# HaiminLuo/svox_t

Hardware: AMD Instinct MI355X
Metric: Mrays/s fwd+bwd, 800×800 render, depth-8 SH9 N3Tree, 1→8 MI355X (higher is better)
Workload: dtype f32

## Files before the change

### svox_t_amd/csrc/svoxt_bwd.hip

```cpp

#include <hip/hip_runtime.h>
#include <stdint.h>

#include "svoxt_launch.h"

#pragma clang fp contract(off)

#include "svoxt_bwd_kernels.h"

using namespace svoxt;

namespace {
int64_t* g_bwd_counters = nullptr;
int64_t* g_bwd_check = nullptr;

template <bool REPLAY>
bool launch_bwd_xform(const TreeDev& tr, const RaysDev& rays, const Opts& opt, int C,
                      const float* grad_out, float* grad, int gstride, RecLists L, const uint4* aux,
                      const float* fwd_out, hipStream_t st) {
    if (opt.format != FMT_SH || C != 3) return false;
    const unsigned nb = nblocks(rays.Q);
#define SVOXT_BWD_XF(BB)                                                                                      \
    hipLaunchKernelGGL((render_bwd_kernel<FMT_SH, 3, BB, true, REPLAY, true>), dim3(nb), dim3(kBlock), 0, st, \
                       tr, rays, opt, grad_out, grad, gstride, L, aux, fwd_out);                         \
    return true;
    switch (opt.basis_dim) {
        case 1: SVOXT_BWD_XF(1)
        case 4: SVOXT_BWD_XF(4)
        case 9: SVOXT_BWD_XF(9)
        case 16: SVOXT_BWD_XF(16)
        case 25: SVOXT_BWD_XF(25)
    }
#undef SVOXT_BWD_XF
    return false;
}

bool launch_lobes_bwd_tiles(const TreeDev& tr, const RaysDev& rays, const Opts& opt, const float* grad_out, float* grad,
                            int gstride, RecLists L, const uint4* aux, hipStream_t st, int terms_state) {
    if (L.terms == nullptr || terms_state != 3 || !lobes_payload(opt, tr.K) || g_bwd_counters != nullptr) return false;
    const unsigned nb = nblocks(rays.Q);
#define SVOXT_LOBES_BWD(BB)                                                                                         \
    {                                                                                                               \
        hipLaunchKernelGGL((render_bwd_kernel<FMT_SH, 3, BB, true, true, false, true, false, true>), dim3(nb), dim3(kBlock), \
                           0, st, tr, rays, opt, grad_out, grad, gstride, L, aux, (const float*)nullptr, (float4*)nullptr); \
        hipLaunchKernelGGL((grad_fused_kernel<FMT_SH, BB, true, false, 3, true>), dim3(nb), dim3(512), 0, st,       \
                           tr, rays, opt, grad_out, L, aux, (const float*)nullptr, grad, gstride);                  \
        return true;                                                                                                \
    }
    switch (opt.basis_dim) {
        case 1: SVOXT_LOBES_BWD(1)
        case 4: SVOXT_LOBES_BWD(4)
        case 9: SVOXT_LOBES_BWD(9)
        case 16: SVOXT_LOBES_BWD(16)
        case 25: SVOXT_LOBES_BWD(25)
    }
#undef SVOXT_LOBES_BWD
    return false;
}

bool launch_bwd_gather(const TreeDev& tr, const RaysDev& rays, const Opts& opt, int C,
                       const float* grad_out, float* grad, int gstride, RecLists L, const uint4* aux,
                       const float* fwd_out, float4* coef, bool xf, hipStream_t st, int terms_state = 0,
                       bool native = false) {
    const unsigned nb = nblocks(rays.Q);
    if (C > 3) {
        if (opt.format != FMT_RGBA || coef != nullptr || xf || fwd_out != nullptr || L.terms == nullptr) return false;
#define SVOXT_WIDE(KK)                                                                                        \
    {                                                                                                         \
        hipLaunchKernelGGL((render_bwd_kernel<FMT_RGBA, KK - 1, 0, true, true, false, true>), dim3(nb), dim3(kBlock), 0, st, \
                           tr, rays, opt, grad_out, grad, gstride, L, aux, (const float*)nullptr, (float4*)nullptr); \
        unsigned long long* ctr = reinterpret_cast<unsigned long long*>(g_bwd_counters);                      \
        unsigned long long* chkw = reinterpret_cast<unsigned long long*>(g_bwd_check);                        \
        if (chkw != nullptr && !native)                                                                       \
            hipLaunchKernelGGL((grad_wide_kernel<KK, false, false, true>), dim3(nb), dim3(512), 0, st, tr, rays, opt, grad_out, L, aux, \
                               grad, gstride, chkw);                                                          \
        else if (chkw != nullptr)                                                                             \
            return false;                                                                                     \
        else if (ctr != nullptr)                                                                              \
// ... 7 lines not shown
                               grad, gstride, (unsigned long long*)nullptr);                                  \
        else                                                                                                  \
            hipLaunchKernelGGL((grad_wide_kernel<KK, false>), dim3(nb), dim3(512), 0, st, tr, rays, opt, grad_out, L, aux, \
                               grad, gstride, (unsigned long long*)nullptr);                                  \
        return true;                                                                                          \
    }
        if (C == 7 && tr.K == 8) SVOXT_WIDE(8)
        if (C == 15 && tr.K == 16) SVOXT_WIDE(16)
        if (C == 31 && tr.K == 32) SVOXT_WIDE(32)
#undef SVOXT_WIDE
        return false;
    }
    if (C != 3) return false;
    const bool fused = coef == nullptr;
    if (fused && xf && (fwd_out != nullptr || opt.format != FMT_SH || opt.basis_dim > 9)) return false;
#define SVOXT_GATHER(F, BB)                                                                                   \
    if (fused) {    \
        hipLaunchKernelGGL((render_bwd_kernel<F, 3, BB, true, true, false, true>), dim3(nb), dim3(kBlock), 0, st, \
                           tr, rays, opt, grad_out, grad, gstride, L, aux, fwd_out, (float4*)nullptr);   \
        unsigned long long* ctr = reinterpret_cast<unsigned long long*>(g_bwd_counters);                      \
        unsigned long long* chkw = reinterpret_cast<unsigned long long*>(g_bwd_check);                        \
        if (chkw != nullptr) {     \
            if (L.terms != nullptr && terms_state == 3 && fwd_out == nullptr)                                 \
                hipLaunchKernelGGL((grad_fused_kernel<F, BB, true, false, 3, false, true>), dim3(nb), dim3(512), 0, st, \
                                   tr, rays, opt, grad_out, L, aux, fwd_out, grad, gstride, chkw);            \
            else if constexpr (F == FMT_SH && BB == 9) {                                                      \
                if (fwd_out != nullptr)                                                                       \
                    hipLaunchKernelGGL((grad_fused_kernel<F, BB, false, false, 0, false, true>), dim3(nb), dim3(512), 0, st, \
                                       tr, rays, opt, grad_out, L, aux, fwd_out, grad, gstride, chkw);        \
                else if (L.terms != nullptr && terms_state == 2)                                              \
                    hipLaunchKernelGGL((grad_fused_kernel<F, BB, true, false, 2, false, true>), dim3(nb), dim3(512), 0, st, \
                                       tr, rays, opt, grad_out, L, aux, fwd_out, grad, gstride, chkw);        \
                else                                                                                          \
                    hipLaunchKernelGGL((grad_fused_kernel<F, BB, true, false, 0, false, true>), dim3(nb), dim3(512), 0, st, \
                                       tr, rays, opt, grad_out, L, aux, fwd_out, grad, gstride, chkw); \
            } else return false;                                                                              \
            return true;                                                                                      \
        }                                                                                                     \
        if (fwd_out != nullptr && ctr == nullptr)                                                             \
            hipLaunchKernelGGL((grad_fused_kernel<F, BB, false>), dim3(nb), dim3(512), 0, st,                 \
                               tr, rays, opt, grad_out, L, aux, fwd_out, grad, gstride);                 \
        else if (ctr == nullptr && L.terms != nullptr && terms_state == 2)                                    \
            hipLaunchKernelGGL((grad_fused_kernel<F, BB, true, false, 2>), dim3(nb), dim3(512), 0, st,        \
                               tr, rays, opt, grad_out, L, aux, fwd_out, grad, gstride);                      \
        else if (ctr == nullptr && L.terms != nullptr && terms_state == 3)                                    \
            hipLaunchKernelGGL((grad_fused_kernel<F, BB, true, false, 3>), dim3(nb), dim3(512), 0, st,        \
                               tr, rays, opt, grad_out, L, aux, fwd_out, grad, gstride);                      \
        else if (ctr == nullptr)            \
            hipLaunchKernelGGL((grad_fused_kernel<F, BB, true>), dim3(nb), dim3(512), 0, st,                  \
                               tr, rays, opt, grad_out, L, aux, fwd_out, grad, gstride);                 \
        else if (fwd_out != nullptr)                                                                          \
            hipLaunchKernelGGL((grad_fused_kernel<F, BB, false, true>), dim3(nb), dim3(512), 0, st,           \
                               tr, rays, opt, grad_out, L, aux, fwd_out, grad, gstride, ctr);            \
        else                                                                                                  \
            hipLaunchKernelGGL((grad_fused_kernel<F, BB, true, true>), dim3(nb), dim3(512), 0, st,            \
                               tr, rays, opt, grad_out, L, aux, fwd_out, grad, gstride, ctr);            \
        return true;                                                                                          \
    }                                                                                                         \
    hipLaunchKernelGGL((render_bwd_kernel<F, 3, BB, true, true, false, true>), dim3(nb), dim3(kBlock), 0, st, \
                       tr, rays, opt, grad_out, grad, gstride, L, aux, fwd_out, coef);                   \
    hipLaunchKernelGGL((grad_merge_kernel<F, BB, 1024, 1024, 4>), dim3(nb), dim3(256), 0, st, tr, rays,      \
                       grad_out, L, coef, aux, grad, gstride);                                                \
    return true;
#define SVOXT_GATHER_XF(BB)                                                                                       \
    hipLaunchKernelGGL((render_bwd_kernel<FMT_SH, 3, BB, true, true, true, true>), dim3(nb), dim3(kBlock), 0, st, \
                       tr, rays, opt, grad_out, grad, gstride, L, aux, fwd_out, coef);                       \
    hipLaunchKernelGGL((grad_merge_kernel<FMT_SH, BB, 1024, 512, 4, true>), dim3(nb), dim3(256), 0, st, tr, rays, \
                       grad_out, L, coef, aux, grad, gstride);                                                    \
    return true;
#define SVOXT_FUSED_XF(BB)                                                                                        \
    {                                                                                                             \
// ... 18 lines not shown
            return false;
        }
        switch (opt.basis_dim) {
            case 1: SVOXT_GATHER_XF(1)
            case 4: SVOXT_GATHER_XF(4)
            case 9: SVOXT_GATHER_XF(9)
        }
        return false;
    }
#undef SVOXT_FUSED_XF
    if (opt.format == FMT_RGBA) { SVOXT_GATHER(FMT_RGBA, 0) }
#define SVOXT_GATHER_WIDE(BB)                                                                                 \
    {                                                                                                         \
        if (!fused || g_bwd_counters != nullptr || fwd_out != nullptr || L.terms == nullptr ||                \
            (terms_state != 2 && terms_state != 3)) return false;                                             \
        hipLaunchKernelGGL((render_bwd_kernel<FMT_SH, 3, BB, true, true, false, true>), dim3(nb), dim3(kBlock), 0, st, \
                           tr, rays, opt, grad_out, grad, gstride, L, aux, fwd_out, (float4*)nullptr);        \
        unsigned long long* chkw = reinterpret_cast<unsigned long long*>(g_bwd_check);                        \
        if (chkw != nullptr && terms_state == 2)                                                              \
            return false;                                                                                     \
        else if (chkw != nullptr)                                                                             \
            hipLaunchKernelGGL((grad_fused_kernel<FMT_SH, BB, true, false, 3, false, true>), dim3(nb), dim3(512), 0, st, \
                               tr, rays, opt, grad_out, L, aux, fwd_out, grad, gstride, chkw);                \
        else if (terms_state == 2)                                                                            \
            hipLaunchKernelGGL((grad_fused_kernel<FMT_SH, BB, true, false, 2>), dim3(nb), dim3(512), 0, st,   \
                               tr, rays, opt, grad_out, L, aux, fwd_out, grad, gstride);                      \
        else                                                                                                  \
            hipLaunchKernelGGL((grad_fused_kernel<FMT_SH, BB, true, false, 3>), dim3(nb), dim3(512), 0, st,   \
                               tr, rays, opt, grad_out, L, aux, fwd_out, grad, gstride);                      \
        return true;                                                                                          \
    }
    if (opt.format == FMT_SH) {
        switch (opt.basis_dim) {
            case 1: SVOXT_GATHER(FMT_SH, 1)
            case 4: SVOXT_GATHER(FMT_SH, 4)
            case 9: SVOXT_GATHER(FMT_SH, 9)
            case 16: SVOXT_GATHER_WIDE(16)
            case 25: SVOXT_GATHER_WIDE(25)
        }
    }
#undef SVOXT_GATHER_WIDE
#undef SVOXT_GATHER
#undef SVOXT_GATHER_XF
    return false;
// ... 107 lines not shown
        }
        else
            done = launch_bwd_xform<false>(tr, rd, od, C, grad_out, grad_features, gs,
                                           dense_lists(S > 0 ? workspace : nullptr, S, rays->Q), nullptr, nullptr, st);
    } else if (C > 0 && full_comp(opt) && !xf)
    {
        const int64_t S = workspace != nullptr ? rec_capacity(workspace_bytes, rays->Q) : 0;
        const RecLists wl = dense_lists(S > 0 ? workspace : nullptr, S, rays->Q);
        if (lists != nullptr) {
            const bool wide = opt->format == SVOXT_FORMAT_RGBA && C > 3;
            const RecLists ll = lists_dev(lists, rays->Q, wide ? 8 : 16);
            const RecLists l1 = wide ? lists_dev(lists, rays->Q, 4) : ll;
            const uint4* laux = reinterpret_cast<const uint4*>(lists->aux);
            if (lobes_payload(od, tree->K)) {
                if (n2 && lists->coef_bytes < 0)
                    done = launch_lobes_bwd_tiles(tr, rd, od, grad_out, grad_features, gs, ll, laux, st, lists->terms_state);
                if (!done) return fail(SVOXT_ERR_UNSUPPORTED, "%s: SG / ASG sample lists serve the per-tile backward only (N = 2, lists.terms filled by the forward: terms_state 3, coef_bytes < 0)", fn);
                return check_launch(fn);
            }
            const bool have_coef = lists->coef != nullptr &&
                                   lists->coef_bytes >= (int64_t)lists->max_samples * rays->Q * 16;
            if (n2 && (tree->K <= 32 || !have_coef) && (have_coef || lists->coef_bytes < 0))
                done = launch_bwd_gather(tr, rd, od, C, grad_out, grad_features, gs, ll, laux,
                                         fwd_out, have_coef ? reinterpret_cast<float4*>(lists->coef) : nullptr, false, st,
                                         (lists->terms_state == 2 || lists->terms_state == 3) ? lists->terms_state : 1,
                                         (lists->flags & SVOXT_LISTS_NATIVE_MATH) != 0);
            if (!done) done = n2 ? launch_bwd_special<true, true>(tr, rd, od, C, grad_out, grad_features, gs, l1, laux, fwd_out, st)
                      : launch_bwd_special<false, true>(tr, rd, od, C, grad_out, grad_features, gs, l1, laux, fwd_out, st);
            if (!done) return fail(SVOXT_ERR_UNSUPPORTED, "%s: no specialised kernel for this payload", fn);
        } else {
            done = n2 ? launch_bwd_special<true, false>(tr, rd, od, C, grad_out, grad_features, gs, wl, nullptr, nullptr, st)
                      : launch_bwd_special<false, false>(tr, rd, od, C, grad_out, grad_features, gs, wl, nullptr, nullptr, st);
        }
    } else if (lists != nullptr) {
        return fail(SVOXT_ERR_UNSUPPORTED, "%s: sample lists need a specialised payload", fn);
    }
    if (!done) {
        const unsigned nb = nblocks(rays->Q);
        const size_t lds = (size_t)(kBlock / 64) * 64 * (tree->K | 1) * sizeof(float) + kBlock * sizeof(int32_t);
        if (C > 0 && lds <= 65536) {
            if (n2) hipLaunchKernelGGL((render_bwd_generic_staged_kernel<true>), dim3(nb), dim3(kBlock), lds, st, tr, rd, od, C, grad_out, grad_features, gs);
// ... 25 lines not shown
```

### svox_t_amd/csrc/svoxt_bwd_kernels.h

```cpp
#pragma once

#include <hip/hip_runtime.h>
#include <stdint.h>

#include "svoxt_device.h"
#include "svoxt_lists.h"

#pragma clang fp contract(off)

#ifndef SVOXT_WIDE_STAGE_ROWS
#define SVOXT_WIDE_STAGE_ROWS 2
#endif
#ifndef SVOXT_WIDE_XCD_ROWS
#define SVOXT_WIDE_XCD_ROWS 1
#endif
#ifndef SVOXT_WIDE_ETAB_WAVES
#define SVOXT_WIDE_ETAB_WAVES 8
#endif

namespace svoxt {



template <int FMT, int C, int BD, int K, bool XF = false>
// ... 180 lines not shown
                  float4* __restrict__ coef_out = nullptr) {
    static_assert(!GATHER || (REPLAY && (C == 3 || FMT == FMT_RGBA)), "per-tile backward: lists; 3 channels or RGBA-style rows");
    static_assert(!ONEPASS || (REPLAY && FMT == FMT_RGBA && !XF && !GATHER), "one sigmoid pass: RGBA-style rows, lists");
    constexpr int K = (FMT == FMT_RGBA) ? (C + 1) : (C * BD + 1);
    constexpr int KS = K | 1;
    __shared__ float stage_all[(kBlock / 64) * 64 * KS];
    __shared__ int32_t sidx_all[kBlock];
    __shared__ uint2 rstage[REPLAY ? 1 : kRecBlock * kBlock];
    __shared__ int32_t ltab[REPLAY ? 1 : kMaxRecBlocks];
    if constexpr (!REPLAY) rec_tab_init(ltab);
    uint2* __restrict__ rec = L.rec;
    const int S = L.S;
    int64_t cur_block = 0;

    if constexpr (GATHER) {
        if (coef_out == nullptr && no_ray_overflowed(L)) return;
    }
    const bool only_overflowed = XF && REPLAY && !GATHER && reinterpret_cast<uintptr_t>(coef_out) == kOnlyOverflowed;
    if (only_overflowed && no_ray_overflowed(L)) return;
    const int lane = threadIdx.x & 63;
    float* stage = stage_all + (threadIdx.x >> 6) * (64 * KS);
    int32_t* sidx = sidx_all + (threadIdx.x >> 6) * 64;
    const unsigned long long lane_lt = (1ull << lane) - 1ull;
    const int64_t tid = (int64_t)blockIdx.x * kBlock + threadIdx.x;
    const int64_t q = ray_of_thread(rays, tid);
    Ray r;
    bool alive = q < rays.Q;
    if (only_overflowed) alive = alive && (aux[alive ? q : 0].x & kRecOverflow) != 0u;
    if constexpr (GATHER) {
        if (coef_out == nullptr && !__any(alive && (aux[alive ? q : 0].x & kRecOverflow) != 0u)) return;
// ... 438 lines not shown
            __builtin_amdgcn_wave_barrier();
        }
        if (k0 + RPP * kRound >= maxn) break;
        __syncthreads();
        for (int i = threadIdx.x; i < T; i += NT) { keys[i] = -1; cnt[i] = 0; }
        if (threadIdx.x == 0) s_nb = 0;
        __syncthreads();
    }
}

template <int FMT, int BD, bool EXACT, bool COUNT = false, int TERMS = 0, bool LOBES = false, bool CHECK = false, bool XF = false>
__global__ void __launch_bounds__(512, 4)
grad_fused_kernel(TreeDev tr, RaysDev rays, Opts opt, const float* __restrict__ grad_out,
                  RecLists L, const uint4* __restrict__ aux, const float* __restrict__ fwd_out,
                  float* __restrict__ grad, int gstride, unsigned long long* __restrict__ counters = nullptr) {
    if (tile_never_recorded(L, blockIdx.x)) return;
#define SVOXT_CHK(i, n, site) chk<CHECK>(i, n, counters, site)
    float4* __restrict__ terms = L.terms;
    constexpr int C = 3, W = 8, P = W - 1, NT = 64 * W, T = 1024, R = (FMT == FMT_SH && BD > 16) ? 896 : 1024;
    static_assert(2 * P * 64 <= R && P >= 1 && P <= W && R <= T, "a pair of rounds must fit the record arrays, a pass the hash table");
    constexpr int K = (FMT == FMT_RGBA) ? (C + 1) : (C * BD + 1);
    constexpr int NB = (FMT == FMT_SH) ? BD : 0;
    constexpr int BDS = (FMT == FMT_SH) ? (BD | 1) : 1;
    constexpr int HALF = K < 16 ? K : 16;
    constexpr int NH = (K + HALF - 1) / HALF;
    constexpr int KS = HALF | 1;
    static_assert(TERMS == 0 || TERMS == 2 || TERMS == 3, "hand-over layouts");
    static_assert(K <= 32 || (EXACT && TERMS >= 2), "wide rows: only with the forward's hand-over (no row in registers)");
    static_assert(!LOBES || (FMT == FMT_SH && EXACT && TERMS >= 2), "lobes: only over the forward's hand-over");
    static_assert(!XF || (FMT == FMT_SH && EXACT && (TERMS == 0 || TERMS == 3) && !LOBES && BD <= 9), "view rotations: SH rows in registers, exact");
    __shared__ float vds[XF ? 64 * 3 : 1];
    __shared__ int32_t keys[T];
    __shared__ int32_t cnt[T];
    __shared__ uint16_t order[R];
    __shared__ uint32_t r_sl[R];
    __shared__ float r_sg[R], r_w[R], r_c[3 * R], r_dt[R];
    __shared__ float bases[64 * BDS];
    __shared__ float gl[64 * 3];
    __shared__ float stage_all[W * 64 * KS];
    __shared__ int32_t seg_all[W * 64];
    __shared__ int32_t s_nb;
    const int lane = threadIdx.x & 63, wave = __builtin_amdgcn_readfirstlane((int)(threadIdx.x >> 6));
    const int pw = wave - (W - P);
    float* stage = stage_all + wave * 64 * KS;
    int32_t* seg = seg_all + wave * 64;
    const int32_t tabreg = rec_tab_reg(L, blockIdx.x, lane);
    const int64_t q = ray_of_thread(rays, (int64_t)blockIdx.x * 64 + lane);
    const bool in_batch = q < rays.Q;
    const int64_t qc = in_batch ? q : 0;
    const bool from_tensors = rays.c2w == nullptr;
    uint4 a = aux[qc];
    float g[C + 1], dsrc[3] = {0.f, 0.f, 1.f}, vsrc[3] = {0.f, 0.f, 1.f};
    if (from_tensors) {
#pragma unroll
        for (int j = 0; j < 3; ++j) dsrc[j] = rays.dirs[3 * qc + j];
        if constexpr (FMT == FMT_SH) {
#pragma unroll
            for (int j = 0; j < 3; ++j) vsrc[j] = rays.vdirs[3 * qc + j];
        }
    }
#pragma unroll
    for (int j = 0; j <= C; ++j) g[j] = grad_out[qc * (C + 1) + j];
    for (int i = threadIdx.x; i < T; i += NT) { keys[i] = -1; cnt[i] = 0; }
    if (!in_batch) a = make_uint4(0u, 0u, 0u, 0u);
    if constexpr (XF) { if (a.x & kRecOverflow) a.x = 0u; }
    const int nrec = (int)(a.x & ~kRecOverflow);
    int maxn = nrec;
    for (int off = 32; off > 0; off >>= 1) maxn = max(maxn, __shfl_xor(maxn, off, 64));
    maxn = __builtin_amdgcn_readfirstlane(maxn);
    if (maxn == 0) return;
    if constexpr (CHECK) { if (threadIdx.x == 0) atomicAdd(counters + kChkBase + 29, 1ull); }

    Ray r;
    float basis[NB > 0 ? NB : 1];
    float accum = 0.f, light = 1.f;
    float light_ray = __uint_as_float(a.z);
    r.delta_scale = 0.f;
    if (from_tensors) {
        float dx, dy, dz;
        r.delta_scale = dir_to_tree(tr, dsrc, dx, dy, dz);
        if constexpr (FMT == FMT_SH && !LOBES && !XF) precalc_basis<BD>(FMT_SH, BD, tr, vsrc[0], vsrc[1], vsrc[2], basis);
    } else if (nrec > 0) {
        setup_ray(tr, rays, opt, q, r);
        if constexpr (FMT == FMT_SH) {
// ... 18 lines not shown
#pragma unroll
            for (int j = 0; j < 3; ++j) vds[lane * 3 + j] = vsrc[j];
        } else {
#pragma unroll
            for (int i = 0; i < NB; ++i) bases[lane * BDS + i] = basis[i];
        }
#pragma unroll
        for (int c = 0; c < C; ++c) gl[lane * 3 + c] = g[c];
    }
    if constexpr (EXACT) {
        float light1 = 1.f;
        const int nr1 = (maxn + P - 1) / P;
        constexpr int D1 = 3;
        float4 tq0 = make_float4(0.f, 0.f, 0.f, 0.f), tq1 = tq0, tq2 = tq0;
        auto terms_at = [&](int k) {
            const int64_t blk = SVOXT_CHK(rec_block_u(L, tabreg, blockIdx.x, k >> 3), L.pool_blocks, 2);
            return terms[TERMS == 2 ? terms_index(blk, lane, k) : terms_index_pm(blk, lane, k)];
        };
        if constexpr (TERMS >= 2) {
            tq0 = terms_at(min(max(pw, 0), maxn - 1));
            tq1 = terms_at(min(max(pw, 0) + P, maxn - 1));
            tq2 = terms_at(min(max(pw, 0) + 2 * P, maxn - 1));
        }
        auto round1 = [&](int rd, float4& tq) {
            const int k = rd * P + pw;
            const float4 tv_cur = tq;
            if (pw >= 0 && rd < nr1 && k < nrec) {
                const int64_t blk = SVOXT_CHK(rec_block_u(L, tabreg, blockIdx.x, k >> 3), L.pool_blocks, 2);
                float att, ex[C];
                if constexpr (TERMS >= 2) {
                    const float4 tv = tv_cur;
                    att = tv.x; ex[0] = tv.y; ex[1] = tv.z; ex[2] = tv.w;
                    if constexpr (XF) {
                        if (k == nrec - 1) {
                            const uint2 e = rec_get(L.rec + rec_index_in(blk, lane, k));
                            rotated_sh_basis<BD>(tr, SVOXT_CHK((int32_t)e.x, tr.M, 6), vsrc, basis);
#pragma unroll
                            for (int i = 0; i < NB; ++i) bases[lane * BDS + i] = basis[i];
                        }
                    }
                } else {
                    const uint2 e = rec_get(L.rec + rec_index_in(blk, lane, k));
                    float row[K];
// ... 59 lines not shown
#pragma unroll
                for (int j = 0; j < C; ++j) total_grad += g[j];
                accum += light1 * opt.background_brightness * total_grad;
                light_ray = light1;
            }
        }
    }
    __syncthreads();

    constexpr bool PRE = EXACT && TERMS != 0;
    constexpr int D2 = 2;
    uint2 eq0 = make_uint2(0u, 0u), eq1 = eq0;
    float4 uq0 = make_float4(0.f, 0.f, 0.f, 0.f), uq1 = uq0;
    auto request = [&](int k, uint2& eq, float4& uq) {
        k = min(max(k, 0), maxn - 1);
        const int64_t blk = SVOXT_CHK(rec_block_u(L, tabreg, blockIdx.x, k >> 3), L.pool_blocks, 2);
        eq = rec_get(L.rec + rec_index_in(blk, lane, k));
        uq = terms[TERMS == 2 ? terms_index(blk, lane, k) : terms_index_pm(blk, lane, k)];
    };
    if constexpr (PRE) {
        request(pw, eq0, uq0);
        request(pw + P, eq1, uq1);
    }
    const unsigned long long lane_lt = (1ull << lane) - 1ull;
    auto round = [&](int kb, int nslot, uint2& eq, float4& uq) -> int {
        int basep[P], total = 0;
        unsigned long long maskp[P];
#pragma unroll
        for (int j = 0; j < P; ++j) {
            maskp[j] = __ballot(nrec > kb + j);
            basep[j] = total;
            total += (int)__popcll(maskp[j]);
        }
        const int k = kb + pw;
        uint2 e = eq;
        const float4 tv_pre = uq;
        if (pw >= 0 && k < nrec) {
            int myb = 0;
            unsigned long long mym = 0ull;
#pragma unroll
            for (int j = 0; j < P; ++j) { if (j == pw) { myb = basep[j]; mym = maskp[j]; } }
            const int slot = SVOXT_CHK(nslot + myb + (int)__popcll(mym & lane_lt), R, 3);
            const int64_t blk = SVOXT_CHK(rec_block_u(L, tabreg, blockIdx.x, k >> 3), L.pool_blocks, 2);
            if constexpr (!PRE) e = rec_get(L.rec + rec_index_in(blk, lane, k));
            float att, tc, cf[C];
            if constexpr (EXACT && TERMS != 0) {
                const float4 tv = tv_pre;
                const float ex[C] = {tv.y, tv.z, tv.w};
                att = tv.x;
                tc = 0.f;
                float row[XF ? K : 1];
                if constexpr (XF) load_row<K>(tr.features + (int64_t)SVOXT_CHK((int32_t)e.x, tr.M, 6) * K, row);
#pragma unroll
                for (int c = 0; c < C; ++c) {
                    const double sd = 1.0 / (1.0 + (double)ex[c]);
                    if constexpr (FMT == FMT_SH) {
                        const float sig = (float)sd;
                        cf[c] = (float)((double)sig * (1.0 - (double)sig));
// ... 708 lines not shown
```

### svox_t_amd/csrc/svoxt_launch.h

```cpp
#pragma once

#include <hip/hip_runtime.h>
#include <stdint.h>

#include "../../include/svoxt.h"
#include "svoxt_device.h"
#include "svoxt_host.h"
#include "svoxt_lists.h"

namespace svoxt {

inline int fail(int code, const char* fmt, const char* a = "", const char* b = "") { return set_error(code, fmt, a, b); }

inline unsigned nblocks(int64_t Q) { return (unsigned)((Q + kBlock - 1) / kBlock); }

inline int64_t rec_rays(int64_t Q) { return (Q + 63) / 64 * 64; }
inline RecLists lists_dev(const svoxt_sample_lists* l, int64_t Q, int term_bytes = 16) {
    RecLists L;
    L.rec = reinterpret_cast<uint2*>(l->rec);
    L.tab = reinterpret_cast<int32_t*>(l->blocktab);
    L.pool_next = reinterpret_cast<int32_t*>(l->pool_next);
    L.pool_blocks = l->blocktab != nullptr ? l->pool_blocks : rec_rays(Q) / 64 * (l->max_samples / kRecBlock);
    L.S = l->max_samples;
    const bool have_terms = l->terms != nullptr && ((uintptr_t)l->terms & 15u) == 0 &&
                            l->terms_bytes >= L.pool_blocks * (int64_t)(64 * kRecBlock) * term_bytes;
    L.terms = have_terms ? reinterpret_cast<float4*>(l->terms) : nullptr;
    return L;
}
inline RecLists dense_lists(void* rec, int64_t S, int64_t Q) {
    RecLists L;
    L.rec = reinterpret_cast<uint2*>(rec);
    L.tab = nullptr;
    L.pool_next = nullptr;
    L.pool_blocks = rec_rays(Q) / 64 * (S / kRecBlock);
    L.S = (int)S;
    L.terms = nullptr;
    return L;
}
inline int64_t rec_capacity(int64_t bytes, int64_t Q) {
    if (bytes <= 0 || Q <= 0) return 0;
    int64_t S = bytes / (8 * rec_rays(Q)) / kRecBlock * kRecBlock;
    return S > 4096 ? 4096 : S;
}

struct Payload { int fmt, C, BD; };

inline bool uses_xform(const svoxt_tree* t, const svoxt_options* o) {
    return t->xform != nullptr && o->format != SVOXT_FORMAT_RGBA;
}

inline bool full_comp(const svoxt_options* o) {
// ... 20 lines not shown
```

### svox_t_amd/csrc/svoxt_lists.h

```cpp
#pragma once

#include <hip/hip_runtime.h>
#include <stdint.h>

#include "svoxt_device.h"

#pragma clang fp contract(off)

namespace svoxt {

constexpr int kBlock = 64;


constexpr uint32_t kRecOverflow = 0x80000000u;
constexpr int kRoleXcds = 8;
__host__ __device__ inline int64_t roles_even(int64_t tiles) { return (tiles + 1) & ~(int64_t)1; }
__host__ __device__ inline int64_t roles_state_words(int64_t tiles) { return roles_even(tiles) + 16 * 32 + (int64_t)kRoleXcds * 2 * tiles; }
constexpr uint32_t kAuxStopped = 1u;

__device__ __forceinline__ void rec_put(uint2* p, uint32_t idx, float delta_t) {
    const unsigned long long v = (unsigned long long)idx | ((unsigned long long)__float_as_uint(delta_t) << 32);
    __builtin_nontemporal_store(v, reinterpret_cast<unsigned long long*>(p));
}
__device__ __forceinline__ uint2 rec_get(const uint2* p) {
// ... 10 lines not shown
    const unsigned long long* q = reinterpret_cast<const unsigned long long*>(p);
    const unsigned long long a = __hip_atomic_load(q, __ATOMIC_RELAXED, __HIP_MEMORY_SCOPE_AGENT);
    const unsigned long long b = __hip_atomic_load(q + 1, __ATOMIC_RELAXED, __HIP_MEMORY_SCOPE_AGENT);
    return make_uint4((uint32_t)a, (uint32_t)(a >> 32), (uint32_t)b, (uint32_t)(b >> 32));
}

constexpr int kRecBlock = 8;
constexpr int kMaxRecBlocks = 64;

struct RecLists {
    uint2* __restrict__ rec;
    int32_t* __restrict__ tab;
    int32_t* __restrict__ pool_next;
    int64_t pool_blocks;
    int S;
    float4* __restrict__ terms;
};
__device__ __forceinline__ int64_t terms_index(int64_t block, int lane, int k) {
    return ((((block << 1) + ((k >> 2) & 1)) << 6) + lane) * 4 + (k & 3);
}
__device__ __forceinline__ int64_t terms_index_pm(int64_t block, int lane, int k) {
    return ((block << 3) + (k & 7)) * 64 + lane;
}

__device__ __forceinline__ int64_t rec_block(const RecLists& L, int64_t tile, int b) {
    const int64_t e = tile * (int64_t)(L.S >> 3) + b;
    return L.tab != nullptr ? (int64_t)L.tab[e] : e;
}
template <bool COHERENT = false>
__device__ __forceinline__ int32_t rec_tab_reg(const RecLists& L, int64_t tile, int lane) {
// ... 14 lines not shown
    if (L.pool_next == nullptr) return false;
    const int32_t* p = L.pool_next + kPoolOverflowWord;
    int32_t w;
    asm volatile("s_load_dword %0, %1, 0x0\n\ts_waitcnt lgkmcnt(0)" : "=s"(w) : "s"(p) : "memory");
    return w != 1;
}
__device__ __forceinline__ bool tile_never_recorded(const RecLists& L, int64_t tile) {
    if (L.tab == nullptr) return false;
    const int32_t* p = L.tab + tile * (int64_t)(L.S >> 3);
    int32_t b0;
    asm volatile("s_load_dword %0, %1, 0x0\n\ts_waitcnt lgkmcnt(0)" : "=s"(b0) : "s"(p) : "memory");
    return b0 == -1;
}
constexpr int kSubPools = 32;
constexpr int kSubPoolStride = 16;
__device__ __forceinline__ int64_t rec_index(const RecLists& L, int64_t tid, int k) {
    return (((rec_block(L, tid >> 6, k >> 3) << 6) + (tid & 63)) << 3) + (k & 7);
}
__device__ __forceinline__ int64_t rec_index_in(int64_t block, int64_t tid, int k) {
    return (((block << 6) + (tid & 63)) << 3) + (k & 7);
}

__device__ __forceinline__ void rec_tab_init(int32_t* ltab) {
    static_assert(kMaxRecBlocks <= 64, "one lane per table entry");
    if ((int)(threadIdx.x & 63) < kMaxRecBlocks) ltab[threadIdx.x & 63] = -1;
    __builtin_amdgcn_fence(__ATOMIC_RELEASE, "wavefront");
    __builtin_amdgcn_wave_barrier();
}
__device__ __forceinline__ int64_t rec_block_begin(const RecLists& L, int32_t* ltab, int64_t tile, int b) {
    if (L.tab == nullptr) return tile * (int64_t)(L.S >> 3) + b;
// ... 96 lines not shown
```

Measured before the change: 1298.

## Dispatch backward gradient tiles from a work list sorted by sample count

Result: slower. 1280, median of 2 (-1.4%).

```diff
diff --git a/exp/trace_tiles.py b/exp/trace_tiles.py
--- /dev/null
+++ b/exp/trace_tiles.py
@@ -0,0 +1,163 @@
+#!/usr/bin/env python3
+import ctypes, os, re, shutil, subprocess, sys, tempfile
+
+ROOT = os.path.dirname(os.path.dirname(os.path.abspath(__file__)))
+SOURCES = ["svoxt_kernels.hip", "svoxt_bwd.hip", "svoxt_build.hip", "svoxt_motion.hip", "svoxt_order.hip", "svoxt_step.hip"]
+SLOTS, TICK_US = 512, 0.01
+
+
+def build(csrc=os.path.join(ROOT, "svox_t_amd", "csrc"), out=os.path.join(ROOT, "exp", "libsvoxt_tiles.so")):
+    tmp = tempfile.mkdtemp()
+    try:
+        shutil.copytree(os.path.join(csrc, "..", "..", "include"), os.path.join(tmp, "include"))
+        dst = os.path.join(tmp, "svox_t_amd", "csrc")
+        shutil.copytree(csrc, dst, ignore=shutil.ignore_patterns("build", "*.so", "*.o", "*.txt", "__pycache__"))
+        p = os.path.join(dst, "svoxt_bwd_kernels.h")
+        s = open(p).read()
+        head = "__global__ void __launch_bounds__(512, 4)\ngrad_fused_kernel(TreeDev tr"
+        assert s.count(head) == 1
+        a = s.index(head)
+        t = s.rindex("template <int FMT, int BD, bool EXACT", 0, a)
+        tmpl = s[t:a].strip()
+        end = s.index("\n}\n", a) + 3
+        body = s[a:end].replace(head, "__device__ __forceinline__ void\ngrad_fused_body(TreeDev tr")
+        mark = "    maxn = __builtin_amdgcn_readfirstlane(maxn);             // everything that decides barriers is scalar\n"
+        assert body.count(mark) == 1
+        tile = "tile" if "int64_t tile = blockIdx.x;" in body else "(int64_t)blockIdx.x"
+        body = body.replace(mark, mark + f"""    if (g_tl != nullptr) {{
+        int s_ = nrec;
+        for (int off = 32; off > 0; off >>= 1) s_ += __shfl_xor(s_, off, 64);
+        if (threadIdx.x == 0) {{
+            g_tl[4 * blockIdx.x + 2] = (unsigned long long){tile};
+            g_tl[4 * blockIdx.x + 3] = ((unsigned long long)maxn << 32) | (unsigned)s_;
+        }}
+    }}
+""")
+        args = re.sub(r"\b(?:int|bool) (\w+)(?: = [^,>]+)?", r"\1", tmpl[len("template <"):-1])
+        wrapper = f"""{tmpl}
+__global__ void __launch_bounds__(512, 4)
+grad_fused_kernel(TreeDev tr, RaysDev rays, Opts opt, const float* __restrict__ grad_out,
+                  RecLists L, const uint4* __restrict__ aux, const float* __restrict__ fwd_out,
+                  float* __restrict__ grad, int gstride, unsigned long long* __restrict__ counters = nullptr) {{
+    const unsigned long long t0 = wall_clock64();
+    grad_fused_body<{args}>(tr, rays, opt, grad_out, L, aux, fwd_out, grad, gstride, counters);
+    __syncthreads();
+    if (threadIdx.x == 0 && g_tl != nullptr) {{ g_tl[4 * blockIdx.x] = t0; g_tl[4 * blockIdx.x + 1] = wall_clock64(); }}
+}}
+"""
+        body_tmpl = re.sub(r" = [^,>]+", "", tmpl)
+        s = s[:t] + "__device__ unsigned long long* g_tl;\n" + body_tmpl + "\n" + body + wrapper + s[end:]
+        open(p, "w").write(s)
+        with open(os.path.join(dst, "svoxt_bwd.hip"), "a") as f:
+            f.write("""
+extern "C" int svoxt_tiles_trace(void* dev_buf) {     // [4 * tiles] u64: start, end, tile, maxn << 32 | records; NULL: off
+    return hipMemcpyToSymbol(HIP_SYMBOL(svoxt::g_tl), &dev_buf, sizeof(void*), 0, hipMemcpyHostToDevice) != hipSuccess;
+}
+""")
+        cmd = ["/opt/rocm/bin/hipcc", "--offload-arch=gfx950", "-O3", "-std=c++17", "-fPIC", "-shared", "-ffp-contract=off",
+               "-fno-fast-math", "-o", os.path.abspath(out)] + [s_ for s_ in SOURCES if os.path.exists(os.path.join(dst, s_))]
+        subprocess.check_call(cmd, cwd=dst)
+    finally:
+        shutil.rmtree(tmp)
+    print(out)
+
+
+def list_schedule(durs, slots=SLOTS):
+    import heapq
+    free = [0.0] * slots
+    heapq.heapify(free)
+    end = 0.0
+    for d in durs:
+        t = heapq.heappop(free) + d
+        end = max(end, t)
+        heapq.heappush(free, t)
+    return end
+
+
+def run(label="this build"):
+    sys.path.insert(0, ROOT)
+    import numpy as np, torch
+    import svox_t_amd as svox, svox_t_amd.csrc as _C
+    from svox_t_amd import synth
+    dev = torch.device("cuda:0")
+    st = synth.shell_tree(8)
+    feats = synth.shell_features(st.n_features, 28).to(dev).requires_grad_(True)
+    tree = svox.N3Tree.from_arrays(st.child, st.data, st.parent_depth, feats.detach(), data_format="SH9", device=dev)
+    r = svox.VolumeRenderer(tree)
+    W = H = 800
+    o, d, v = synth.pinhole_rays(W, H)
+    rays = svox.Rays(o.to(dev), d.to(dev), v.to(dev))
+    gout = synth.grad_output(W * H, 4).to(dev)
+    ntiles = (W * H + 63) // 64
+    buf = torch.full((ntiles * 4,), -1, dtype=torch.int64, device=dev)
+    lib = _C._lib
+    lib.svoxt_tiles_trace.argtypes = [ctypes.c_void_p]
+
+    def step():
+        feats.grad = None
+        r(feats, rays, image_shape=(H, W)).backward(gout)
+
+    for _ in range(30):
+        step()
+    torch.cuda.synchronize()
+    reps = []
+    for rep in range(3):
+        buf.fill_(-1)
+        assert lib.svoxt_tiles_trace(ctypes.c_void_p(buf.data_ptr())) == 0
+        step()
+        torch.cuda.synchronize()
+        assert lib.svoxt_tiles_trace(None) == 0
+        reps.append(buf.view(ntiles, 4).cpu().numpy().astype(np.int64))
+    print(f"== {label}: route {_C.LAST_ROUTE['backward']}")
+    for rep, e in enumerate(reps):
+        report(e, rep, np)
+
+
+def report(e, rep, np):
+    t0, t1 = e[:, 0], e[:, 1]
+    real = e[:, 2] >= 0
+    maxn = np.where(real, e[:, 3] >> 32, 0)
+    recs = np.where(real, e[:, 3] & 0xFFFFFFFF, 0)
+    base = t0.min()
+    s, f = (t0 - base) * TICK_US, (t1 - base) * TICK_US
+    dur = f - s
+    span = f.max()
+    print(f"-- run {rep}: {len(e)} workgroups, {real.sum()} on tiles with samples; kernel span {span:.1f} us "
+          f"(first start -> last end)")
+    print(f"   slot-time: {dur.sum():.0f} slot-us in all ({dur.sum() / SLOTS:.1f} us over {SLOTS} slots); "
+          f"empty workgroups {dur[~real].sum():.0f} slot-us ({dur[~real].sum() / dur.sum():.1%}; "
+          f"{dur[~real].mean() if (~real).any() else 0:.2f} us each)")
+    last_real_start = s[real].max() if real.any() else 0.0
+    print(f"   tail: last start of a tile with samples at {last_real_start:.1f} us, kernel end {span:.1f} us "
+          f"-> {span - last_real_start:.1f} us; longest tile {dur[real].max():.1f} us, median {np.median(dur[real]):.1f} us")
+    step = max(span / 20, 1e-3)
+    line = []
+    for k in range(20):
+        a, b = k * step, (k + 1) * step
+        res = ((np.minimum(f, b) - np.maximum(s, a)).clip(0)).sum() / step
+        line.append(f"{res:4.0f}")
+    print(f"   resident workgroups per {step:.1f} us: " + " ".join(line))
+    if real.sum() > 2:
+        c1 = np.corrcoef(np.ceil(maxn[real] / 7), dur[real])[0, 1]
+        x = np.stack([np.ceil(maxn[real] / 7), recs[real] / 64, np.ones(real.sum())], 1)
+        coef, *_ = np.linalg.lstsq(x, dur[real], rcond=None)
+        c2 = np.corrcoef(x @ coef, dur[real])[0, 1]
+        print(f"   duration vs ceil(maxn / 7): r = {c1:.3f}; vs a fit of ceil(maxn / 7) and records / 64: r = {c2:.3f} "
+              f"({coef[0]:.2f} us per round, {coef[1]:.2f} us per record per ray, {coef[2]:.2f} us)")
+    order_now = np.argsort(t0, kind="stable")
+    tile_order = np.argsort(np.where(real, e[:, 2], 1 << 40), kind="stable")
+    sims = {
+        "(a) as dispatched, every workgroup": dur[order_now],
+        "(b) tiles with samples only, image order": dur[tile_order][: real.sum()],
+        "(c) tiles with samples, longest (measured) first": np.sort(dur[real])[::-1],
+        "(d) tiles with samples, maxn buckets of 8 first (the work list)": dur[real][np.argsort(-(np.minimum((maxn[real] - 1) // 8, 15)), kind="stable")],
+    }
+    for name, dd in sims.items():
+        print(f"   list scheduling at {SLOTS} slots {name}: {list_schedule(dd):.1f} us")
+
+
+if __name__ == "__main__":
+    if sys.argv[1] == "build":
+        build(*sys.argv[2:])
+    else:
+        run(*sys.argv[2:])
diff --git a/svox_t_amd/csrc/svoxt_bwd.hip b/svox_t_amd/csrc/svoxt_bwd.hip
--- a/svox_t_amd/csrc/svoxt_bwd.hip
+++ b/svox_t_amd/csrc/svoxt_bwd.hip
@@ -36,9 +36,11 @@
 }
 
 bool launch_lobes_bwd_tiles(const TreeDev& tr, const RaysDev& rays, const Opts& opt, const float* grad_out, float* grad,
-                            int gstride, RecLists L, const uint4* aux, hipStream_t st, int terms_state) {
-    if (L.terms == nullptr || terms_state != 3 || !lobes_payload(opt, tr.K) || g_bwd_counters != nullptr) return false;
+                            int gstride, RecLists L0, const uint4* aux, hipStream_t st, int terms_state,
+                            const svoxt_sample_lists* lists) {
+    if (L0.terms == nullptr || terms_state != 3 || !lobes_payload(opt, tr.K) || g_bwd_counters != nullptr) return false;
     const unsigned nb = nblocks(rays.Q);
+    const RecLists L = with_work_list(L0, lists, rays.Q);
 #define SVOXT_LOBES_BWD(BB)                                                                                         \
     {                                                                                                               \
         hipLaunchKernelGGL((render_bwd_kernel<FMT_SH, 3, BB, true, true, false, true, false, true>), dim3(nb), dim3(kBlock), \
@@ -61,7 +63,7 @@
 bool launch_bwd_gather(const TreeDev& tr, const RaysDev& rays, const Opts& opt, int C,
                        const float* grad_out, float* grad, int gstride, RecLists L, const uint4* aux,
                        const float* fwd_out, float4* coef, bool xf, hipStream_t st, int terms_state = 0,
-                       bool native = false) {
+                       bool native = false, const svoxt_sample_lists* lists = nullptr) {
     const unsigned nb = nblocks(rays.Q);
     if (C > 3) {
         if (opt.format != FMT_RGBA || coef != nullptr || xf || fwd_out != nullptr || L.terms == nullptr) return false;
@@ -99,47 +101,51 @@
     if (C != 3) return false;
     const bool fused = coef == nullptr;
     if (fused && xf && (fwd_out != nullptr || opt.format != FMT_SH || opt.basis_dim > 9)) return false;
+    const RecLists Lw = (fused && !xf) ? with_work_list(L, lists, rays.Q) : L;
 #define SVOXT_GATHER(F, BB)                                                                                   \
     if (fused) {    \
+                  \
+        const bool unchecked = g_bwd_check != nullptr && !(L.terms != nullptr && terms_state == 3 && fwd_out == nullptr) && \
+                               !(F == FMT_SH && BB == 9);                                                     \
         hipLaunchKernelGGL((render_bwd_kernel<F, 3, BB, true, true, false, true>), dim3(nb), dim3(kBlock), 0, st, \
-                           tr, rays, opt, grad_out, grad, gstride, L, aux, fwd_out, (float4*)nullptr);   \
+                           tr, rays, opt, grad_out, grad, gstride, unchecked ? L : Lw, aux, fwd_out, (float4*)nullptr); \
         unsigned long long* ctr = reinterpret_cast<unsigned long long*>(g_bwd_counters);                      \
         unsigned long long* chkw = reinterpret_cast<unsigned long long*>(g_bwd_check);                        \
         if (chkw != nullptr) {     \
             if (L.terms != nullptr && terms_state == 3 && fwd_out == nullptr)                                 \
                 hipLaunchKernelGGL((grad_fused_kernel<F, BB, true, false, 3, false, true>), dim3(nb), dim3(512), 0, st, \
-                                   tr, rays, opt, grad_out, L, aux, fwd_out, grad, gstride, chkw);            \
+                                   tr, rays, opt, grad_out, Lw, aux, fwd_out, grad, gstride, chkw);            \
             else if constexpr (F == FMT_SH && BB == 9) {                                                      \
                 if (fwd_out != nullptr)                                                                       \
                     hipLaunchKernelGGL((grad_fused_kernel<F, BB, false, false, 0, false, true>), dim3(nb), dim3(512), 0, st, \
-                                       tr, rays, opt, grad_out, L, aux, fwd_out, grad, gstride, chkw);        \
+                                       tr, rays, opt, grad_out, Lw, aux, fwd_out, grad, gstride, chkw);        \
                 else if (L.terms != nullptr && terms_state == 2)                                              \
                     hipLaunchKernelGGL((grad_fused_kernel<F, BB, true, false, 2, false, true>), dim3(nb), dim3(512), 0, st, \
-                                       tr, rays, opt, grad_out, L, aux, fwd_out, grad, gstride, chkw);        \
+                                       tr, rays, opt, grad_out, Lw, aux, fwd_out, grad, gstride, chkw);        \
                 else                                                                                          \
                     hipLaunchKernelGGL((grad_fused_kernel<F, BB, true, false, 0, false, true>), dim3(nb), dim3(512), 0, st, \
-                                       tr, rays, opt, grad_out, L, aux, fwd_out, grad, gstride, chkw); \
+                                       tr, rays, opt, grad_out, Lw, aux, fwd_out, grad, gstride, chkw); \
             } else return false;                                                                              \
             return true;                                                                                      \
         }                                                                                                     \
         if (fwd_out != nullptr && ctr == nullptr)                                                             \
             hipLaunchKernelGGL((grad_fused_kernel<F, BB, false>), dim3(nb), dim3(512), 0, st,                 \
-                               tr, rays, opt, grad_out, L, aux, fwd_out, grad, gstride);                 \
+                               tr, rays, opt, grad_out, Lw, aux, fwd_out, grad, gstride);                 \
         else if (ctr == nullptr && L.terms != nullptr && terms_state == 2)                                    \
             hipLaunchKernelGGL((grad_fused_kernel<F, BB, true, false, 2>), dim3(nb), dim3(512), 0, st,        \
-                               tr, rays, opt, grad_out, L, aux, fwd_out, grad, gstride);                      \
+                               tr, rays, opt, grad_out, Lw, aux, fwd_out, grad, gstride);                      \
         else if (ctr == nullptr && L.terms != nullptr && terms_state == 3)                                    \
             hipLaunchKernelGGL((grad_fused_kernel<F, BB, true, false, 3>), dim3(nb), dim3(512), 0, st,        \
-                               tr, rays, opt, grad_out, L, aux, fwd_out, grad, gstride);                      \
+                               tr, rays, opt, grad_out, Lw, aux, fwd_out, grad, gstride);                      \
         else if (ctr == nullptr)            \
             hipLaunchKernelGGL((grad_fused_kernel<F, BB, true>), dim3(nb), dim3(512), 0, st,                  \
-                               tr, rays, opt, grad_out, L, aux, fwd_out, grad, gstride);                 \
+                               tr, rays, opt, grad_out, Lw, aux, fwd_out, grad, gstride);                 \
         else if (fwd_out != nullptr)                                                                          \
             hipLaunchKernelGGL((grad_fused_kernel<F, BB, false, true>), dim3(nb), dim3(512), 0, st,           \
-                               tr, rays, opt, grad_out, L, aux, fwd_out, grad, gstride, ctr);            \
+                               tr, rays, opt, grad_out, Lw, aux, fwd_out, grad, gstride, ctr);            \
         else                                                                                                  \
             hipLaunchKernelGGL((grad_fused_kernel<F, BB, true, true>), dim3(nb), dim3(512), 0, st,            \
-                               tr, rays, opt, grad_out, L, aux, fwd_out, grad, gstride, ctr);            \
+                               tr, rays, opt, grad_out, Lw, aux, fwd_out, grad, gstride, ctr);            \
         return true;                                                                                          \
     }                                                                                                         \
     hipLaunchKernelGGL((render_bwd_kernel<F, 3, BB, true, true, false, true>), dim3(nb), dim3(kBlock), 0, st, \
@@ -188,20 +194,21 @@
     {                                                                                                         \
         if (!fused || g_bwd_counters != nullptr || fwd_out != nullptr || L.terms == nullptr ||                \
             (terms_state != 2 && terms_state != 3)) return false;                                             \
+        unsigned long long* chkw = reinterpret_cast<unsigned long long*>(g_bwd_check);                        \
         hipLaunchKernelGGL((render_bwd_kernel<FMT_SH, 3, BB, true, true, false, true>), dim3(nb), dim3(kBlock), 0, st, \
-                           tr, rays, opt, grad_out, grad, gstride, L, aux, fwd_out, (float4*)nullptr);        \
-        unsigned long long* chkw = reinterpret_cast<unsigned long long*>(g_bwd_check);                        \
+                           tr, rays, opt, grad_out, grad, gstride, (chkw != nullptr && terms_state == 2) ? L : Lw, aux, \
+                           fwd_out, (float4*)nullptr);                                                        \
         if (chkw != nullptr && terms_state == 2)                                                              \
             return false;                                                                                     \
         else if (chkw != nullptr)                                                                             \
             hipLaunchKernelGGL((grad_fused_kernel<FMT_SH, BB, true, false, 3, false, true>), dim3(nb), dim3(512), 0, st, \
-                               tr, rays, opt, grad_out, L, aux, fwd_out, grad, gstride, chkw);                \
+                               tr, rays, opt, grad_out, Lw, aux, fwd_out, grad, gstride, chkw);                \
         else if (terms_state == 2)                                                                            \
             hipLaunchKernelGGL((grad_fused_kernel<FMT_SH, BB, true, false, 2>), dim3(nb), dim3(512), 0, st,   \
-                               tr, rays, opt, grad_out, L, aux, fwd_out, grad, gstride);                      \
+                               tr, rays, opt, grad_out, Lw, aux, fwd_out, grad, gstride);                      \
         else                                                                                                  \
             hipLaunchKernelGGL((grad_fused_kernel<FMT_SH, BB, true, false, 3>), dim3(nb), dim3(512), 0, st,   \
-                               tr, rays, opt, grad_out, L, aux, fwd_out, grad, gstride);                      \
+                               tr, rays, opt, grad_out, Lw, aux, fwd_out, grad, gstride);                      \
         return true;                                                                                          \
     }
     if (opt.format == FMT_SH) {
@@ -339,7 +346,7 @@
             const uint4* laux = reinterpret_cast<const uint4*>(lists->aux);
             if (lobes_payload(od, tree->K)) {
                 if (n2 && lists->coef_bytes < 0)
-                    done = launch_lobes_bwd_tiles(tr, rd, od, grad_out, grad_features, gs, ll, laux, st, lists->terms_state);
+                    done = launch_lobes_bwd_tiles(tr, rd, od, grad_out, grad_features, gs, ll, laux, st, lists->terms_state, lists);
                 if (!done) return fail(SVOXT_ERR_UNSUPPORTED, "%s: SG / ASG sample lists serve the per-tile backward only (N = 2, lists.terms filled by the forward: terms_state 3, coef_bytes < 0)", fn);
                 return check_launch(fn);
             }
@@ -349,7 +356,7 @@
                 done = launch_bwd_gather(tr, rd, od, C, grad_out, grad_features, gs, ll, laux,
                                          fwd_out, have_coef ? reinterpret_cast<float4*>(lists->coef) : nullptr, false, st,
                                          (lists->terms_state == 2 || lists->terms_state == 3) ? lists->terms_state : 1,
-                                         (lists->flags & SVOXT_LISTS_NATIVE_MATH) != 0);
+                                         (lists->flags & SVOXT_LISTS_NATIVE_MATH) != 0, lists);
             if (!done) done = n2 ? launch_bwd_special<true, true>(tr, rd, od, C, grad_out, grad_features, gs, l1, laux, fwd_out, st)
                       : launch_bwd_special<false, true>(tr, rd, od, C, grad_out, grad_features, gs, l1, laux, fwd_out, st);
             if (!done) return fail(SVOXT_ERR_UNSUPPORTED, "%s: no specialised kernel for this payload", fn);
diff --git a/svox_t_amd/csrc/svoxt_bwd_kernels.h b/svox_t_amd/csrc/svoxt_bwd_kernels.h
--- a/svox_t_amd/csrc/svoxt_bwd_kernels.h
+++ b/svox_t_amd/csrc/svoxt_bwd_kernels.h
@@ -218,6 +218,12 @@
     int64_t cur_block = 0;
 
     if constexpr (GATHER) {
+        if (coef_out == nullptr && L.work_off != 0 && !tile_never_recorded(L, blockIdx.x)) {
+            const int64_t qw = ray_of_thread(rays, (int64_t)blockIdx.x * kBlock + threadIdx.x);
+            int n = qw < rays.Q ? (int)(aux[qw].x & ~kRecOverflow) : 0;
+            for (int off = 32; off > 0; off >>= 1) n = max(n, __shfl_xor(n, off, 64));
+            if (threadIdx.x == 0 && n > 0) work_list_append(L, blockIdx.x, gridDim.x, n);
+        }
         if (coef_out == nullptr && no_ray_overflowed(L)) return;
     }
     const bool only_overflowed = XF && REPLAY && !GATHER && reinterpret_cast<uintptr_t>(coef_out) == kOnlyOverflowed;
@@ -686,8 +692,15 @@
 grad_fused_kernel(TreeDev tr, RaysDev rays, Opts opt, const float* __restrict__ grad_out,
                   RecLists L, const uint4* __restrict__ aux, const float* __restrict__ fwd_out,
                   float* __restrict__ grad, int gstride, unsigned long long* __restrict__ counters = nullptr) {
-    if (tile_never_recorded(L, blockIdx.x)) return;
 #define SVOXT_CHK(i, n, site) chk<CHECK>(i, n, counters, site)
+    int64_t tile = blockIdx.x;
+    int wl_total = 0, wl_ticket = 0;
+    if (L.work_off != 0) {
+        tile = work_list_tile(L, blockIdx.x, gridDim.x, wl_total);
+        if (tile < 0) return;
+        tile = SVOXT_CHK(tile, (int64_t)gridDim.x, 14);
+        if (threadIdx.x == 0) wl_ticket = work_list_ticket(L);
+    } else if (tile_never_recorded(L, tile)) return;
     float4* __restrict__ terms = L.terms;
     constexpr int C = 3, W = 8, P = W - 1, NT = 64 * W, T = 1024, R = (FMT == FMT_SH && BD > 16) ? 896 : 1024;
     static_assert(2 * P * 64 <= R && P >= 1 && P <= W && R <= T, "a pair of rounds must fit the record arrays, a pass the hash table");
@@ -716,8 +729,8 @@
     const int pw = wave - (W - P);
     float* stage = stage_all + wave * 64 * KS;
     int32_t* seg = seg_all + wave * 64;
-    const int32_t tabreg = rec_tab_reg(L, blockIdx.x, lane);
-    const int64_t q = ray_of_thread(rays, (int64_t)blockIdx.x * 64 + lane);
+    const int32_t tabreg = rec_tab_reg(L, tile, lane);
+    const int64_t q = ray_of_thread(rays, tile * 64 + lane);
     const bool in_batch = q < rays.Q;
     const int64_t qc = in_batch ? q : 0;
     const bool from_tensors = rays.c2w == nullptr;
@@ -740,6 +753,7 @@
     int maxn = nrec;
     for (int off = 32; off > 0; off >>= 1) maxn = max(maxn, __shfl_xor(maxn, off, 64));
     maxn = __builtin_amdgcn_readfirstlane(maxn);
+    if (L.work_off != 0 && threadIdx.x == 0) work_list_done(L, wl_ticket, wl_total);
     if (maxn == 0) return;
     if constexpr (CHECK) { if (threadIdx.x == 0) atomicAdd(counters + kChkBase + 29, 1ull); }
 
@@ -788,7 +802,7 @@
         constexpr int D1 = 3;
         float4 tq0 = make_float4(0.f, 0.f, 0.f, 0.f), tq1 = tq0, tq2 = tq0;
         auto terms_at = [&](int k) {
-            const int64_t blk = SVOXT_CHK(rec_block_u(L, tabreg, blockIdx.x, k >> 3), L.pool_blocks, 2);
+            const int64_t blk = SVOXT_CHK(rec_block_u(L, tabreg, tile, k >> 3), L.pool_blocks, 2);
             return terms[TERMS == 2 ? terms_index(blk, lane, k) : terms_index_pm(blk, lane, k)];
         };
         if constexpr (TERMS >= 2) {
@@ -800,7 +814,7 @@
             const int k = rd * P + pw;
             const float4 tv_cur = tq;
             if (pw >= 0 && rd < nr1 && k < nrec) {
-                const int64_t blk = SVOXT_CHK(rec_block_u(L, tabreg, blockIdx.x, k >> 3), L.pool_blocks, 2);
+                const int64_t blk = SVOXT_CHK(rec_block_u(L, tabreg, tile, k >> 3), L.pool_blocks, 2);
                 float att, ex[C];
                 if constexpr (TERMS >= 2) {
                     const float4 tv = tv_cur;
@@ -890,7 +904,7 @@
     float4 uq0 = make_float4(0.f, 0.f, 0.f, 0.f), uq1 = uq0;
     auto request = [&](int k, uint2& eq, float4& uq) {
         k = min(max(k, 0), maxn - 1);
-        const int64_t blk = SVOXT_CHK(rec_block_u(L, tabreg, blockIdx.x, k >> 3), L.pool_blocks, 2);
+        const int64_t blk = SVOXT_CHK(rec_block_u(L, tabreg, tile, k >> 3), L.pool_blocks, 2);
         eq = rec_get(L.rec + rec_index_in(blk, lane, k));
         uq = terms[TERMS == 2 ? terms_index(blk, lane, k) : terms_index_pm(blk, lane, k)];
     };
@@ -917,7 +931,7 @@
 #pragma unroll
             for (int j = 0; j < P; ++j) { if (j == pw) { myb = basep[j]; mym = maskp[j]; } }
             const int slot = SVOXT_CHK(nslot + myb + (int)__popcll(mym & lane_lt), R, 3);
-            const int64_t blk = SVOXT_CHK(rec_block_u(L, tabreg, blockIdx.x, k >> 3), L.pool_blocks, 2);
+            const int64_t blk = SVOXT_CHK(rec_block_u(L, tabreg, tile, k >> 3), L.pool_blocks, 2);
             if constexpr (!PRE) e = rec_get(L.rec + rec_index_in(blk, lane, k));
             float att, tc, cf[C];
             if constexpr (EXACT && TERMS != 0) {
diff --git a/svox_t_amd/csrc/svoxt_launch.h b/svox_t_amd/csrc/svoxt_launch.h
--- a/svox_t_amd/csrc/svoxt_launch.h
+++ b/svox_t_amd/csrc/svoxt_launch.h
@@ -25,6 +25,17 @@
     const bool have_terms = l->terms != nullptr && ((uintptr_t)l->terms & 15u) == 0 &&
                             l->terms_bytes >= L.pool_blocks * (int64_t)(64 * kRecBlock) * term_bytes;
     L.terms = have_terms ? reinterpret_cast<float4*>(l->terms) : nullptr;
+    L.work_off = 0;
+    return L;
+}
+inline RecLists with_work_list(RecLists L, const svoxt_sample_lists* l, int64_t Q) {
+    if (l == nullptr || l->blocktab == nullptr || l->pool_next == nullptr || l->tile_state == nullptr) return L;
+    const int64_t tiles = rec_rays(Q) / 64;
+    static_assert(kWorkBuckets <= 2 * kRoleXcds && kWorkBuckets < kSubPools, "the ready queues hold the lists, pool_next's parts the counters");
+    const intptr_t lists = reinterpret_cast<intptr_t>(l->tile_state) + (intptr_t)(roles_even(tiles) + 16 * 32) * 4;
+    const int64_t off = (int64_t)(lists - reinterpret_cast<intptr_t>(l->pool_next)) / 4;
+    if (off != (int64_t)(int32_t)off || off == 0) return L;
+    L.work_off = (int32_t)off;
     return L;
 }
 inline RecLists dense_lists(void* rec, int64_t S, int64_t Q) {
@@ -35,6 +46,7 @@
     L.pool_blocks = rec_rays(Q) / 64 * (S / kRecBlock);
     L.S = (int)S;
     L.terms = nullptr;
+    L.work_off = 0;
     return L;
 }
 inline int64_t rec_capacity(int64_t bytes, int64_t Q) {
diff --git a/svox_t_amd/csrc/svoxt_lists.h b/svox_t_amd/csrc/svoxt_lists.h
--- a/svox_t_amd/csrc/svoxt_lists.h
+++ b/svox_t_amd/csrc/svoxt_lists.h
@@ -48,6 +48,7 @@
     int32_t* __restrict__ pool_next;
     int64_t pool_blocks;
     int S;
+    int work_off;
     float4* __restrict__ terms;
 };
 __device__ __forceinline__ int64_t terms_index(int64_t block, int lane, int k) {
@@ -92,6 +93,45 @@
 }
 constexpr int kSubPools = 32;
 constexpr int kSubPoolStride = 16;
+constexpr int kWorkBuckets = 16;
+constexpr int kWorkBucketWidth = 8;
+constexpr int kWorkCtrWord = 2;
+__device__ __forceinline__ int32_t* work_lists(const RecLists& L) { return L.pool_next + L.work_off; }
+__device__ __forceinline__ int32_t* work_ctr(const RecLists& L) { return L.pool_next + kWorkCtrWord; }
+__device__ __forceinline__ int work_bucket(int maxn ) {
+    const int b = (maxn - 1) / kWorkBucketWidth;
+    return kWorkBuckets - 1 - (b < kWorkBuckets - 1 ? b : kWorkBuckets - 1);
+}
+__device__ __forceinline__ void work_list_append(const RecLists& L, int64_t tile, int64_t ntiles, int maxn) {
+    const int b = work_bucket(maxn);
+    const int pos = atomicAdd(work_ctr(L) + b * kSubPoolStride, 1) + 1;
+    work_lists(L)[b * ntiles + pos] = (int32_t)tile;
+}
+__device__ __forceinline__ int64_t work_list_tile(const RecLists& L, int64_t b, int64_t ntiles, int& total) {
+    const int lane = (int)(threadIdx.x & 63);
+    int c = 0;
+    if (lane < kWorkBuckets) c = work_ctr(L)[lane * kSubPoolStride] + 1;
+    int incl = c;
+#pragma unroll
+    for (int off = 1; off < kWorkBuckets; off <<= 1) {
+        const int v = __shfl_up(incl, off, 64);
+        if (lane >= off) incl += v;
+    }
+    total = __builtin_amdgcn_readlane(incl, kWorkBuckets - 1);
+    if (b >= total) return -1;
+    const unsigned long long before = __ballot(lane < kWorkBuckets && (int64_t)incl <= b);
+    const int j = __popcll(before);
+    const int start = j > 0 ? __builtin_amdgcn_readlane(incl, j - 1) : 0;
+    return (int64_t)__builtin_amdgcn_readfirstlane(work_lists(L)[j * ntiles + (b - start)]);
+}
+__device__ __forceinline__ int work_list_ticket(const RecLists& L) {
+    return atomicAdd(work_ctr(L) + kWorkBuckets * kSubPoolStride, 1);
+}
+__device__ __forceinline__ void work_list_done(const RecLists& L, int ticket, int total) {
+    if (ticket != total - 2) return;
+#pragma unroll
+    for (int j = 0; j <= kWorkBuckets; ++j) work_ctr(L)[j * kSubPoolStride] = -1;
+}
 __device__ __forceinline__ int64_t rec_index(const RecLists& L, int64_t tid, int k) {
     return (((rec_block(L, tid >> 6, k >> 3) << 6) + (tid & 63)) << 3) + (k & 7);
 }
```
